# yongkyung-oh/Stable-Neural-SDEs

Measured on AMD Instinct MI355X. Metric: SDE solver steps/sec (batch x steps / s), forward solve, higher is better.
Workload: dtype f32; 1 GPU; K2: Neural LNSDE (io=4,no=17) NL=2 B=1024/GPU H=128 C=21 L=101 natural-spline coeffs 30% NaN, 100 Euler steps dt=1, ts=[0,100], in-kernel Philox dW; rows_per_gpu=1024, solver_steps=100, global_rows=1024, parallelism=row-shard x1, no collective in the solver, kernel=auto, prepare=every call (weight pack + time table launch inside the timed region, as r01-r04)

## Files before the change

stable-neural-sdes_amd/csrc/snsde_m4_kernel.h:

```cpp
#pragma once
#include <type_traits>

#include "snsde_mfma_kernels.h"

namespace snsde_mfma {

template <int H_, int NHID_, int KUXT_, int YIN_, int SAVE_, int ACT_ = 0, int ACC_ = 0>
struct CfgL {
    static constexpr bool ACC = ACC_ != 0;
    static constexpr bool SWISH = ACT_ != 0;
    static constexpr int H = H_, NHID = NHID_, KUXT = KUXT_;
    static constexpr bool YIN = YIN_ != 0;
    static constexpr bool SAVE = SAVE_ != 0;
    static constexpr int NW = H / 16;
    static constexpr int NT = NW * 64;
    static constexpr int WPS = NW >= 4 ? NW / 4 : 1;
    static constexpr int KUH = H / 16;
    static constexpr int LDY = ld_for(16 * KUH, 16);
    static constexpr int LDX = ld_for(16 * (KUXT > 0 ? KUXT : 1), 16);
    static constexpr int LDA = LDY;
    static constexpr int NLAYER = NHID + 2;
    static constexpr int NSAVE = NHID + 2 + (SWISH ? NHID + 1 : 0);
    static constexpr int ZSLOT = NHID + 1;
    static constexpr int PRE0 = NHID + 2;
    static constexpr int ZB = 4;
    static constexpr int ZSTASH = 4 * ZB * 64;
    static constexpr int ROWCH = 128;
    static constexpr int XI = KUXT > 0 ? (4 * 16 * KUXT + NT - 1) / NT : 1;
    static constexpr int RS = 8;
    static constexpr int ACCF = 64;
    static constexpr int LDS_FLOATS = 4 * (LDY + 2 * LDX + 2 * LDA) + (ROWCH + 3) * RS + NW * ZSTASH + ACCF;
};

template <bool NANZ>
__device__ __forceinline__ float lean_tanh(float x) {
    const float t = __builtin_amdgcn_exp2f(fabsf(x) * -2.8853900817779268f);
    float q = (1.0f - t) * __builtin_amdgcn_rcpf(1.0f + t);
    if constexpr (NANZ) q = __builtin_fmaxf(q, 0.0f);
    return __builtin_copysignf(q, x);
}

template <bool NANZ>
__device__ __forceinline__ float lean_tanh_rel(float x) {
    const float x2 = x * x;
    float p = fmaf(x2, -0.053968253968253971f, 0.13333333333333333f);
    p = fmaf(x2, p, -0.33333333333333333f);
    p = fmaf(x * x2, p, x);
    const float q = lean_tanh<NANZ>(x);
    return fabsf(x) < 0.125f ? p : q;
}

__device__ __forceinline__ float lean_swish(float x, float scale) {
    const float e = __builtin_amdgcn_exp2f(x * -1.4426950408889634f);
    return (x * scale) * __builtin_amdgcn_rcpf(1.0f + e);
}

template <int KU>
__device__ __forceinline__ void lean_load_w(float (&w)[KU * 4], const float* __restrict__ g, int wave, int lane) {
#pragma unroll
    for (int u = 0; u < KU; ++u) {
        const f32x4 v = *reinterpret_cast<const f32x4*>(g + (((size_t)wave * KU + u) * 64 + lane) * 4);
        w[4 * u] = v[0]; w[4 * u + 1] = v[1]; w[4 * u + 2] = v[2]; w[4 * u + 3] = v[3];
    }
}

__device__ __forceinline__ void lean_gload(float& dst, uint32_t voff, const float* sbase) {
    asm volatile("s_nop 4\n\tglobal_load_dword %0, %1, %2" : "=v"(dst) : "v"(voff), "s"(lean_uniform(sbase)) : "memory");
}
__device__ __forceinline__ void lean_gstore(float v, uint32_t voff, const float* sbase) {
    asm volatile("s_nop 4\n\tglobal_store_dword %1, %0, %2" :: "v"(v), "v"(voff), "s"(lean_uniform(sbase)));
}
__device__ __forceinline__ void lean_gload4(float& d0, float& d1, float& d2, float& d3, uint32_t v0, uint32_t v1, uint32_t v2,
                                            uint32_t v3, const float* sbase) {
    asm volatile("s_nop 4\n\tglobal_load_dword %0, %4, %8\n\tglobal_load_dword %1, %5, %8\n\tglobal_load_dword %2, %6, %8\n\t"
                 "global_load_dword %3, %7, %8"
                 : "=&v"(d0), "=&v"(d1), "=&v"(d2), "=&v"(d3) : "v"(v0), "v"(v1), "v"(v2), "v"(v3), "s"(lean_uniform(sbase)) : "memory");
}
template <int KU> struct LeanB { f32x4 v[KU]; };
__device__ __forceinline__ void lean_read_b(uint32_t a, LeanB<1>& b) {
    asm volatile("s_mov_b64 exec, 0xffff\n\tds_read_b128 %0, %[a]\n\ts_mov_b64 exec, -1" : "=&v"(b.v[0]) : [a] "v"(a));
}
__device__ __forceinline__ void lean_read_b(uint32_t a, LeanB<2>& b) {
    asm volatile("s_mov_b64 exec, 0xffff\n\tds_read_b128 %0, %[a]\n\tds_read_b128 %1, %[a] offset:64\n\ts_mov_b64 exec, -1"
                 : "=&v"(b.v[0]), "=&v"(b.v[1]) : [a] "v"(a));
}
__device__ __forceinline__ void lean_read_b(uint32_t a, LeanB<3>& b) {
    asm volatile("s_mov_b64 exec, 0xffff\n\tds_read_b128 %0, %[a]\n\tds_read_b128 %1, %[a] offset:64\n\tds_read_b128 %2, %[a] offset:128\n\t"
                 "s_mov_b64 exec, -1" : "=&v"(b.v[0]), "=&v"(b.v[1]), "=&v"(b.v[2]) : [a] "v"(a));
}
__device__ __forceinline__ void lean_read_b(uint32_t a, LeanB<4>& b) {
    asm volatile("s_mov_b64 exec, 0xffff\n\tds_read_b128 %0, %[a]\n\tds_read_b128 %1, %[a] offset:64\n\tds_read_b128 %2, %[a] offset:128\n\t"
                 "ds_read_b128 %3, %[a] offset:192\n\ts_mov_b64 exec, -1"
                 : "=&v"(b.v[0]), "=&v"(b.v[1]), "=&v"(b.v[2]), "=&v"(b.v[3]) : [a] "v"(a));
}
__device__ __forceinline__ void lean_read_b(uint32_t a, LeanB<5>& b) {
    asm volatile("s_mov_b64 exec, 0xffff\n\tds_read_b128 %0, %[a]\n\tds_read_b128 %1, %[a] offset:64\n\tds_read_b128 %2, %[a] offset:128\n\t"
                 "ds_read_b128 %3, %[a] offset:192\n\tds_read_b128 %4, %[a] offset:256\n\ts_mov_b64 exec, -1"
                 : "=&v"(b.v[0]), "=&v"(b.v[1]), "=&v"(b.v[2]), "=&v"(b.v[3]), "=&v"(b.v[4]) : [a] "v"(a));
}
__device__ __forceinline__ void lean_read_b(uint32_t a, LeanB<6>& b) {
    asm volatile("s_mov_b64 exec, 0xffff\n\tds_read_b128 %0, %[a]\n\tds_read_b128 %1, %[a] offset:64\n\tds_read_b128 %2, %[a] offset:128\n\t"
                 "ds_read_b128 %3, %[a] offset:192\n\tds_read_b128 %4, %[a] offset:256\n\tds_read_b128 %5, %[a] offset:320\n\t"
                 "s_mov_b64 exec, -1"
                 : "=&v"(b.v[0]), "=&v"(b.v[1]), "=&v"(b.v[2]), "=&v"(b.v[3]), "=&v"(b.v[4]), "=&v"(b.v[5]) : [a] "v"(a));
}
__device__ __forceinline__ void lean_read_b(uint32_t a, LeanB<8>& b) {
    asm volatile("s_mov_b64 exec, 0xffff\n\tds_read_b128 %0, %[a]\n\tds_read_b128 %1, %[a] offset:64\n\tds_read_b128 %2, %[a] offset:128\n\t"
                 "ds_read_b128 %3, %[a] offset:192\n\tds_read_b128 %4, %[a] offset:256\n\tds_read_b128 %5, %[a] offset:320\n\t"
                 "ds_read_b128 %6, %[a] offset:384\n\tds_read_b128 %7, %[a] offset:448\n\ts_mov_b64 exec, -1"
                 : "=&v"(b.v[0]), "=&v"(b.v[1]), "=&v"(b.v[2]), "=&v"(b.v[3]), "=&v"(b.v[4]), "=&v"(b.v[5]), "=&v"(b.v[6]), "=&v"(b.v[7])
                 : [a] "v"(a));
}
__device__ __forceinline__ void lean_read_b_carried(uint32_t a, LeanB<1>& b) {
    asm volatile("s_mov_b64 exec, 0xffff\n\tds_read_b128 %0, %[a]\n\ts_mov_b64 exec, -1" : "+v"(b.v[0]) : [a] "v"(a));
}
__device__ __forceinline__ void lean_read_b_carried(uint32_t a, LeanB<2>& b) {
    asm volatile("s_mov_b64 exec, 0xffff\n\tds_read_b128 %0, %[a]\n\tds_read_b128 %1, %[a] offset:64\n\ts_mov_b64 exec, -1"
                 : "+v"(b.v[0]), "+v"(b.v[1]) : [a] "v"(a));
}
__device__ __forceinline__ void lean_read_b_carried(uint32_t a, LeanB<3>& b) {
    asm volatile("s_mov_b64 exec, 0xffff\n\tds_read_b128 %0, %[a]\n\tds_read_b128 %1, %[a] offset:64\n\tds_read_b128 %2, %[a] offset:128\n\t"
                 "s_mov_b64 exec, -1" : "+v"(b.v[0]), "+v"(b.v[1]), "+v"(b.v[2]) : [a] "v"(a));
}
__device__ __forceinline__ void lean_read_b_carried(uint32_t a, LeanB<4>& b) {
    asm volatile("s_mov_b64 exec, 0xffff\n\tds_read_b128 %0, %[a]\n\tds_read_b128 %1, %[a] offset:64\n\tds_read_b128 %2, %[a] offset:128\n\t"
                 "ds_read_b128 %3, %[a] offset:192\n\ts_mov_b64 exec, -1"
                 : "+v"(b.v[0]), "+v"(b.v[1]), "+v"(b.v[2]), "+v"(b.v[3]) : [a] "v"(a));
}
__device__ __forceinline__ void lean_read_b_carried(uint32_t a, LeanB<5>& b) {
    asm volatile("s_mov_b64 exec, 0xffff\n\tds_read_b128 %0, %[a]\n\tds_read_b128 %1, %[a] offset:64\n\tds_read_b128 %2, %[a] offset:128\n\t"
                 "ds_read_b128 %3, %[a] offset:192\n\tds_read_b128 %4, %[a] offset:256\n\ts_mov_b64 exec, -1"
                 : "+v"(b.v[0]), "+v"(b.v[1]), "+v"(b.v[2]), "+v"(b.v[3]), "+v"(b.v[4]) : [a] "v"(a));
}
__device__ __forceinline__ void lean_read_b_carried(uint32_t a, LeanB<6>& b) {
    asm volatile("s_mov_b64 exec, 0xffff\n\tds_read_b128 %0, %[a]\n\tds_read_b128 %1, %[a] offset:64\n\tds_read_b128 %2, %[a] offset:128\n\t"
                 "ds_read_b128 %3, %[a] offset:192\n\tds_read_b128 %4, %[a] offset:256\n\tds_read_b128 %5, %[a] offset:320\n\t"
                 "s_mov_b64 exec, -1"
                 : "+v"(b.v[0]), "+v"(b.v[1]), "+v"(b.v[2]), "+v"(b.v[3]), "+v"(b.v[4]), "+v"(b.v[5]) : [a] "v"(a));
}
__device__ __forceinline__ void lean_read_b_carried(uint32_t a, LeanB<8>& b) {
    asm volatile("s_mov_b64 exec, 0xffff\n\tds_read_b128 %0, %[a]\n\tds_read_b128 %1, %[a] offset:64\n\tds_read_b128 %2, %[a] offset:128\n\t"
                 "ds_read_b128 %3, %[a] offset:192\n\tds_read_b128 %4, %[a] offset:256\n\tds_read_b128 %5, %[a] offset:320\n\t"
                 "ds_read_b128 %6, %[a] offset:384\n\tds_read_b128 %7, %[a] offset:448\n\ts_mov_b64 exec, -1"
                 : "+v"(b.v[0]), "+v"(b.v[1]), "+v"(b.v[2]), "+v"(b.v[3]), "+v"(b.v[4]), "+v"(b.v[5]), "+v"(b.v[6]), "+v"(b.v[7])
                 : [a] "v"(a));
}
#undef SNSDE_RD
template <int CNT> __device__ __forceinline__ void lean_wait2(f32x4& x, f32x4& y) {
    asm volatile("s_waitcnt lgkmcnt(%2)" : "+v"(x), "+v"(y) : "n"(CNT < 15 ? CNT : 15));
}
template <int CNT> __device__ __forceinline__ void lean_wait1(f32x4& x) {
    asm volatile("s_waitcnt lgkmcnt(%1)" : "+v"(x) : "n"(CNT < 15 ? CNT : 15));
}
template <int Y, int KU, int U>
__device__ __forceinline__ void lean_gemm_from(const float (&w)[KU * 4], LeanB<KU>& b, f32x4& c, f32x4& d) {
    if constexpr (U < KU) {
        if constexpr (U + 1 < KU) lean_wait2<Y + KU - 2 - U>(b.v[U], b.v[U + 1]);
        else lean_wait1<Y>(b.v[U]);
#pragma unroll
        for (int uu = U; uu < U + 2 && uu < KU; ++uu) {
            c = __builtin_amdgcn_mfma_f32_4x4x1f32(w[4 * uu], b.v[uu][0], c, 0, 0, 4);
            d = __builtin_amdgcn_mfma_f32_4x4x1f32(w[4 * uu + 1], b.v[uu][1], d, 0, 0, 4);
            c = __builtin_amdgcn_mfma_f32_4x4x1f32(w[4 * uu + 2], b.v[uu][2], c, 0, 0, 4);
            d = __builtin_amdgcn_mfma_f32_4x4x1f32(w[4 * uu + 3], b.v[uu][3], d, 0, 0, 4);
        }
        __builtin_amdgcn_sched_barrier(0);
        lean_gemm_from<Y, KU, U + 2>(w, b, c, d);
    }
}
template <int Y, int KU>
__device__ __forceinline__ void lean_gemm(const float (&w)[KU * 4], LeanB<KU>& b, f32x4& c, f32x4& d) {
    lean_gemm_from<Y, KU, 0>(w, b, c, d);
}

typedef short s16x4 __attribute__((ext_vector_type(4)));
typedef __bf16 bf16x4 __attribute__((ext_vector_type(4)));
template <class CF> struct CfgBf16 : CF { static constexpr bool BF = true; };
template <class CF, class = void> struct lean_bf : std::false_type {};
template <class CF> struct lean_bf<CF, std::void_t<decltype(CF::BF)>> : std::bool_constant<CF::BF> {};
template <int KU> struct LeanBh { s16x4 v[KU]; };
template <bool BF, int KU> using LeanWt = std::conditional_t<BF, s16x4[KU], float[KU * 4]>;
template <bool BF, int KU> using LeanBt = std::conditional_t<BF, LeanBh<KU>, LeanB<KU>>;
template <bool BF> using LeanOp = std::conditional_t<BF, __bf16, float>;

__device__ __forceinline__ s16x4 lean_bf16x4(f32x4 v) {
    const bf16x4 b = {(__bf16)v[0], (__bf16)v[1], (__bf16)v[2], (__bf16)v[3]};
    return __builtin_bit_cast(s16x4, b);
}
template <int KU>
__device__ __forceinline__ void lean_load_w(s16x4 (&w)[KU], const float* __restrict__ g, int wave, int lane) {
#pragma unroll
    for (int u = 0; u < KU; ++u) w[u] = lean_bf16x4(*reinterpret_cast<const f32x4*>(g + (((size_t)wave * KU + u) * 64 + lane) * 4));
}
template <bool BF>
__device__ __forceinline__ uint32_t lean_op_addr(const float* buf, int roff, int col) {
    if constexpr (BF) return lean_lds_addr(buf) + (uint32_t)((roff + col) * 2);
    else return lean_lds_addr(buf + roff + col);
}
#define LEAN_RB(i, o) "\n\tds_read_b64 %" #i ", %[a] offset:" #o
#define LEAN_RB_PRE "s_mov_b64 exec, 0xffff"
#define LEAN_RB_POST "\n\ts_mov_b64 exec, -1"
__device__ __forceinline__ void lean_read_b(uint32_t a, LeanBh<1>& b) {
    asm volatile(LEAN_RB_PRE LEAN_RB(0, 0) LEAN_RB_POST : "=&v"(b.v[0]) : [a] "v"(a));
}
__device__ __forceinline__ void lean_read_b(uint32_t a, LeanBh<2>& b) {
    asm volatile(LEAN_RB_PRE LEAN_RB(0, 0) LEAN_RB(1, 32) LEAN_RB_POST : "=&v"(b.v[0]), "=&v"(b.v[1]) : [a] "v"(a));
}
__device__ __forceinline__ void lean_read_b(uint32_t a, LeanBh<3>& b) {
    asm volatile(LEAN_RB_PRE LEAN_RB(0, 0) LEAN_RB(1, 32) LEAN_RB(2, 64) LEAN_RB_POST
                 : "=&v"(b.v[0]), "=&v"(b.v[1]), "=&v"(b.v[2]) : [a] "v"(a));
}
__device__ __forceinline__ void lean_read_b(uint32_t a, LeanBh<4>& b) {
    asm volatile(LEAN_RB_PRE LEAN_RB(0, 0) LEAN_RB(1, 32) LEAN_RB(2, 64) LEAN_RB(3, 96) LEAN_RB_POST
                 : "=&v"(b.v[0]), "=&v"(b.v[1]), "=&v"(b.v[2]), "=&v"(b.v[3]) : [a] "v"(a));
}
__device__ __forceinline__ void lean_read_b(uint32_t a, LeanBh<6>& b) {
    asm volatile(LEAN_RB_PRE LEAN_RB(0, 0) LEAN_RB(1, 32) LEAN_RB(2, 64) LEAN_RB(3, 96) LEAN_RB(4, 128) LEAN_RB(5, 160) LEAN_RB_POST
                 : "=&v"(b.v[0]), "=&v"(b.v[1]), "=&v"(b.v[2]), "=&v"(b.v[3]), "=&v"(b.v[4]), "=&v"(b.v[5]) : [a] "v"(a));
}
__device__ __forceinline__ void lean_read_b(uint32_t a, LeanBh<8>& b) {
    asm volatile(LEAN_RB_PRE LEAN_RB(0, 0) LEAN_RB(1, 32) LEAN_RB(2, 64) LEAN_RB(3, 96) LEAN_RB(4, 128) LEAN_RB(5, 160)
                 LEAN_RB(6, 192) LEAN_RB(7, 224) LEAN_RB_POST
                 : "=&v"(b.v[0]), "=&v"(b.v[1]), "=&v"(b.v[2]), "=&v"(b.v[3]), "=&v"(b.v[4]), "=&v"(b.v[5]), "=&v"(b.v[6]),
                   "=&v"(b.v[7]) : [a] "v"(a));
}
__device__ __forceinline__ void lean_read_b_carried(uint32_t a, LeanBh<1>& b) {
    asm volatile(LEAN_RB_PRE LEAN_RB(0, 0) LEAN_RB_POST : "+v"(b.v[0]) : [a] "v"(a));
}
__device__ __forceinline__ void lean_read_b_carried(uint32_t a, LeanBh<2>& b) {
    asm volatile(LEAN_RB_PRE LEAN_RB(0, 0) LEAN_RB(1, 32) LEAN_RB_POST : "+v"(b.v[0]), "+v"(b.v[1]) : [a] "v"(a));
}
__device__ __forceinline__ void lean_read_b_carried(uint32_t a, LeanBh<3>& b) {
    asm volatile(LEAN_RB_PRE LEAN_RB(0, 0) LEAN_RB(1, 32) LEAN_RB(2, 64) LEAN_RB_POST
                 : "+v"(b.v[0]), "+v"(b.v[1]), "+v"(b.v[2]) : [a] "v"(a));
}
__device__ __forceinline__ void lean_read_b_carried(uint32_t a, LeanBh<6>& b) {
    asm volatile(LEAN_RB_PRE LEAN_RB(0, 0) LEAN_RB(1, 32) LEAN_RB(2, 64) LEAN_RB(3, 96) LEAN_RB(4, 128) LEAN_RB(5, 160) LEAN_RB_POST
                 : "+v"(b.v[0]), "+v"(b.v[1]), "+v"(b.v[2]), "+v"(b.v[3]), "+v"(b.v[4]), "+v"(b.v[5]) : [a] "v"(a));
}
#undef LEAN_RB
#undef LEAN_RB_PRE
#undef LEAN_RB_POST
template <int CNT> __device__ __forceinline__ void lean_wait2(s16x4& x, s16x4& y) {
    asm volatile("s_waitcnt lgkmcnt(%2)" : "+v"(x), "+v"(y) : "n"(CNT < 15 ? CNT : 15));
}
template <int CNT> __device__ __forceinline__ void lean_wait1(s16x4& x) {
    asm volatile("s_waitcnt lgkmcnt(%1)" : "+v"(x) : "n"(CNT < 15 ? CNT : 15));
}
template <int Y, int KU, int U>
__device__ __forceinline__ void lean_gemm_from(const s16x4 (&w)[KU], LeanBh<KU>& b, f32x4& c, f32x4& d) {
    if constexpr (U < KU) {
        if constexpr (U + 1 < KU) lean_wait2<Y + KU - 2 - U>(b.v[U], b.v[U + 1]);
        else lean_wait1<Y>(b.v[U]);
        c = __builtin_amdgcn_mfma_f32_4x4x4bf16_1k(w[U], b.v[U], c, 0, 0, 4);
        if constexpr (U + 1 < KU) d = __builtin_amdgcn_mfma_f32_4x4x4bf16_1k(w[U + 1], b.v[U + 1], d, 0, 0, 4);
        __builtin_amdgcn_sched_barrier(0);
        lean_gemm_from<Y, KU, U + 2>(w, b, c, d);
    }
}
template <int Y, int KU>
__device__ __forceinline__ void lean_gemm(const s16x4 (&w)[KU], LeanBh<KU>& b, f32x4& c, f32x4& d) {
    lean_gemm_from<Y, KU, 0>(w, b, c, d);
}

template <class CF, int GEO_> struct CfgSpec : CF {
    static constexpr bool SPEC = true, SPEC_GEO = GEO_ != 0;
    static constexpr int XB = 4;
    static constexpr int LDS_FLOATS = CF::LDS_FLOATS + 4 * (XB - 2) * CF::LDX;
    static_assert(CF::XI == 1 && 4 * 16 * CF::KUXT <= 16 * CF::NW && CF::ROWCH % XB == 0, "CfgSpec: one spline entry per lane, 16 lanes per step of a batch");
};
template <class CF, class = void> struct lean_spec : std::false_type {};
template <class CF> struct lean_spec<CF, std::void_t<decltype(CF::SPEC)>> : std::bool_constant<CF::SPEC> {};
template <class CF> constexpr int lean_xslots() {
    if constexpr (lean_spec<CF>::value) return CF::XB;
    else return 2;
}
template <class CF> constexpr bool lean_spec_geo() {
    if constexpr (lean_spec<CF>::value) return CF::SPEC_GEO;
    else return false;
}

#ifdef LEAN_TRACE
#define LT_DECL unsigned long long lt[10]; uint32_t* const ltl = reinterpret_cast<uint32_t*>(lds + CF::LDS_FLOATS) + tid; \
    if constexpr (!BF) { for (int i_ = 0; i_ < 12; ++i_) ltl[i_ * NT] = 0u; }
#define LT(i) if constexpr (!BF) { asm volatile("s_memtime %0" : "=s"(lt[i])); }
#define LT_ADD(slot, i) __hip_atomic_fetch_add(ltl + (slot) * NT, (uint32_t)lt[i], __ATOMIC_RELAXED, __HIP_MEMORY_SCOPE_WORKGROUP);
#define LT_COLLECT_A if constexpr (!BF) { asm volatile("s_waitcnt lgkmcnt(0)" : "+s"(lt[0]), "+s"(lt[1]), "+s"(lt[2]), "+s"(lt[3])); \
    LT_ADD(0, 0) LT_ADD(1, 1) LT_ADD(2, 2) LT_ADD(3, 3) if (n > 0) LT_ADD(10, 0) }
#define LT_COLLECT_B if constexpr (!BF) { asm volatile("s_waitcnt lgkmcnt(0)" : "+s"(lt[4]), "+s"(lt[5]), "+s"(lt[6])); LT_ADD(4, 4) LT_ADD(5, 5) LT_ADD(6, 6) }
#define LT_COLLECT if constexpr (!BF) { asm volatile("s_waitcnt lgkmcnt(0)" : "+s"(lt[7]), "+s"(lt[8]), "+s"(lt[9])); LT_ADD(7, 7) LT_ADD(8, 8) LT_ADD(9, 9) \
    if (n + 1 < N) LT_ADD(11, 9) }
#define LT_LDS_EXTRA (12 * CF::NT * sizeof(uint32_t))
#else
#define LT_DECL
#define LT(i)
#define LT_COLLECT_A
#define LT_COLLECT_B
#define LT_COLLECT
#define LT_LDS_EXTRA 0
#endif

#ifdef LEAN_KNOCKOUT
#define LEAN_KO(SP) (SP)
#else
#define LEAN_KO(SP) false
#endif
#if (defined(LEAN_KNOCKOUT) || defined(LEAN_SPEC_WPS)) && !defined(SNSDE_DEV_SUBSET)
#error "LEAN_KNOCKOUT / LEAN_SPEC_WPS are development switches (build.py variant): never part of a product build"
#endif
#ifndef LEAN_SPEC_WPS
#define LEAN_SPEC_WPS CF::WPS
#endif

#ifndef LEAN_TANH_F
#define LEAN_TANH_F lean_tanh_rel<false>
#endif
#ifndef LEAN_TANH_G
#define LEAN_TANH_G lean_tanh_rel<true>
#endif

template <class CF>
__global__ void __launch_bounds__(CF::NT, lean_spec<CF>::value ? LEAN_SPEC_WPS : CF::WPS) snsde_m4_kernel(MfmaArgs a) {
    constexpr int H = CF::H, NT = CF::NT, NHID = CF::NHID, KUH = CF::KUH, KUXT = CF::KUXT;
    constexpr int LDY = CF::LDY, LDX = CF::LDX, LDA = CF::LDA, RS = CF::RS;
    constexpr bool YIN = CF::YIN, SAVE = CF::SAVE;
    constexpr bool BF = lean_bf<CF>::value;
    constexpr bool SP = lean_spec<CF>::value;
    static_assert(!SP || (!BF && !CF::ACC && !CF::SWISH && KUXT > 0 && 16 * KUXT + 16 <= LDX), "CfgSpec: f32 relu fields with a control path");
    using OpT = LeanOp<BF>;
    extern __shared__ __attribute__((aligned(16))) float lds[];
    float* ybuf = lds;
    constexpr int XS = lean_xslots<CF>();
    float* xbuf = ybuf + 4 * LDY;
    float* bufA = xbuf + 4 * XS * LDX;
    float* bufB = bufA + 4 * LDA;
    float* rowtab = bufB + 4 * LDA;
    float* zstash_all = rowtab + (CF::ROWCH + 3) * RS;
    float* accbuf = zstash_all + CF::NW * CF::ZSTASH;

    const int tid = threadIdx.x;
    const int lane = tid & 63;
    const int wave = __builtin_amdgcn_readfirstlane(tid >> 6);
    const int r = lane & 3, s = (lane >> 2) & 3, q = lane >> 4;
    const int fo = wave * 16 + 4 * q + s;
    const int row0 = blockIdx.x * 4;
    const int B = a.B, C = a.C, N = a.N;
    const int row = row0 + r;
    const bool row_ok = row < B;
    const int rowc = row_ok ? row : B - 1;
    const size_t BH = (size_t)B * H;
    const size_t goff = (size_t)rowc * H + fo;
    float* zstash = zstash_all + wave * CF::ZSTASH;
    const uint32_t fo4 = (uint32_t)(fo * sizeof(float)), goff4 = (uint32_t)(goff * sizeof(float));
    const int xc = a.lean_xc;
    const bool time_on = a.lean_time != 0, geo = SP ? lean_spec_geo<CF>() : a.lean_geo != 0;
    const float act_scale = a.act == SNSDE_ACT_LIPSWISH ? 0.909f : 1.0f;
    const int f_out = SP ? (int)SNSDE_DRIFT_TANH : a.f_out;
    const bool g_raw = !SP && a.g_out == SNSDE_DIFFUSION_RAW;

    int li = 0;
    LeanWt<BF, (KUXT > 0 ? KUXT : 1)> wxt;
    LeanWt<BF, KUH> wy, wh[NHID > 0 ? NHID : 1], wo;
    if constexpr (KUXT > 0) lean_load_w<KUXT>(wxt, a.ws + a.w_off[li++], wave, lane);
    if constexpr (YIN) lean_load_w<KUH>(wy, a.ws + a.w_off[li++], wave, lane);
#pragma unroll
    for (int l = 0; l < NHID; ++l) lean_load_w<KUH>(wh[l], a.ws + a.w_off[li++], wave, lane);
    lean_load_w<KUH>(wo, a.ws + a.w_off[li++], wave, lane);
    f32x4 bfr[CF::NLAYER];
#pragma unroll
    for (int l = 0; l < CF::NLAYER; ++l)
#pragma unroll
        for (int i = 0; i < 4; ++i) bfr[l][i] = (s == 0) ? a.ws[a.bias_off + l * H + wave * 16 + 4 * q + i] : 0.0f;

    for (int i = tid; i < 4 * (LDY + XS * LDX + 2 * LDA); i += NT) lds[i] = 0.0f;
    auto fill_rows = [&](int base) {
        for (int i = tid; i < (CF::ROWCH + 3) * RS; i += NT) {
            const int j = i % RS;
            int rr = base + i / RS + (j == 0 ? 0 : (j == 7 ? 2 : 1));
            rr = rr < N - 1 ? rr : N - 1;
            const int src = j == 0 ? 1 : j == 1 ? 6 : j == 4 ? (a.raw_time ? 0 : 2) : j == 5 ? (a.raw_time ? 10 : 3) : j == 6 ? 4 : j == 7 ? 5 : 10;
            rowtab[i] = a.step_tab[(size_t)rr * SNSDE_STEP_STRIDE + src];
        }
    };
    fill_rows(0);
    __syncthreads();

    const float sig_theta = snsde_sigmoid(a.params[a.off_theta]);
    const int no = a.no;
    const bool tab = SP || a.gt_off >= 0;
    const float* gt = a.gt_ext ? a.gt_ext : a.ws + (tab ? a.gt_off : 0);
    const bool mul_y = SP || (no == 13 || no == 17 || no == 3 || no == 6 || no == 11);
    const bool yfun = !SP && (no >= 7 && no <= 10);
    const bool mil = !SP && a.method == SNSDE_MILSTEIN;
    const bool phx = SP || a.dW == nullptr;
    const uint32_t grow = (uint32_t)(a.row_offset + row);
    const uint64_t seed = a.seed_dev ? *a.seed_dev : a.seed;
    const int rslot = a.row_out ? a.row_out[rowc] : -1;

    float yv = a.y0[goff];
    reinterpret_cast<OpT*>(ybuf)[r * LDY + fo] = (OpT)yv;
    if (row_ok) {
        a.ys[(size_t)row * H + fo] = yv;
        if constexpr (SAVE) { if (a.traj) a.traj[(size_t)row * H + fo] = yv; }
    }

    const int xw = xc + (time_on ? 2 : 0);
    const int xquota = (4 * xw + CF::NW - 1) / CF::NW;
    float ca[CF::XI], cb[CF::XI], cc[CF::XI], cd[CF::XI];
    uint32_t cvo[CF::XI];
    int xdst[CF::XI], xkind[CF::XI];
    const size_t cstride = (size_t)(a.L - 1) * 4 * C;
    [[maybe_unused]] const int xslot = SP ? ((1 + q) & 3) * (4 * LDX) : 0;
#pragma unroll
    for (int i = 0; i < CF::XI; ++i) {
        const int li_ = SP ? (lane & 15) : lane + 64 * i, it = wave * xquota + li_;
        const bool ok = KUXT > 0 && li_ < xquota && it < 4 * xw;
        const int rr = ok ? it / xw : 0, col = ok ? it - rr * xw : 0;
        xdst[i] = ok ? rr * LDX + col : (SP ? (lane & 3) * LDX + 16 * KUXT + (lane >> 2) : -1);
        xkind[i] = col < xc ? 0 : (col == xc ? 1 : 2);
        const int gr = row0 + rr < B ? rr : B - 1 - row0, ch = col < xc ? col : 0;
        cvo[i] = (uint32_t)((gr * cstride + ch) * sizeof(float));
    }
    const bool has_x = SP || (KUXT > 0 && xc > 0);
    const float* ctile = a.coeffs + (size_t)row0 * cstride;
    const uint32_t cstep = (uint32_t)(C * sizeof(float));
    const uint32_t cidx = (uint32_t)(4 * C * sizeof(float));
    auto load_coeffs = [&](int idx) {
        if (__builtin_expect(has_x, 1)) {
            const uint32_t io = (uint32_t)idx * cidx;
#pragma unroll
            for (int i = 0; i < CF::XI; ++i)
                lean_gload4(ca[i], cb[i], cc[i], cd[i], cvo[i] + io, cvo[i] + io + cstep, cvo[i] + io + 2 * cstep,
                            cvo[i] + io + 3 * cstep, ctile);
        }
    };
    auto vm_wait = [&](float& dwn, float& gtn) {
        asm volatile("s_waitcnt vmcnt(0)" : "+v"(dwn), "+v"(gtn));
#pragma unroll
        for (int i = 0; i < CF::XI; ++i) asm volatile("" : "+v"(ca[i]), "+v"(cb[i]), "+v"(cc[i]), "+v"(cd[i]));
    };
    auto store_xt = [&](float* xb, float frac, float sn, float cs) {
        if constexpr (KUXT > 0) {
#pragma unroll
            for (int i = 0; i < CF::XI; ++i) {
                float v = 0.0f;
                if (__builtin_expect(has_x, 1)) {
                    const float x3 = cd[i] * frac;
                    float q3 = x3 * 0.333333343f;
                    q3 = fmaf(fmaf(-3.0f, q3, x3), 0.333333343f, q3);
                    v = ca[i] + (cb[i] + (0.5f * cc[i] + q3) * frac) * frac;
                }
                v = xkind[i] == 0 ? v : (xkind[i] == 1 ? sn : cs);
                if (SP || xdst[i] >= 0) reinterpret_cast<OpT*>(xb)[xdst[i]] = (OpT)v;
            }
        }
    };

    auto next_dw = [&](int i, float sqh) -> float {
        if (__builtin_expect(phx, 1)) {
            const int k = (int)((uint32_t)i % (uint32_t)(4 * CF::ZB));
            if (__builtin_expect(k == 0 && !(LEAN_KO(SP) && i > 0), 0)) {
                float zq[4 * CF::ZB];
#pragma unroll
                for (int bb = 0; bb < CF::ZB; ++bb)
                    snsde_philox_normal4(seed, grow, (uint32_t)((i >> 2) + bb), (uint32_t)fo, &zq[4 * bb]);
#pragma unroll
                for (int j = 0; j < 4 * CF::ZB; ++j) zstash[j * 64 + lane] = zq[j];
            }
            return zstash[k * 64 + lane] * sqh;
        }
        float v;
        lean_gload(v, goff4, a.dW + (size_t)i * BH);
        return v;
    };

    auto gpart = [&](float y, float gtv, float dwv, float hh) -> float {
        float g = 0.0f, draw = 0.0f;
        if (__builtin_expect(yfun, 0)) {
            float p1, p2;
            const float raw = snsde_phi(no, y, p1, p2);
            g = fast_tanh(sig_theta * snsde_nan_to_num(raw));
            draw = snsde_finite(raw) ? p1 : 0.0f;
        } else
        {
            const float raw = mul_y ? gtv * y : gtv;
            if (__builtin_expect(g_raw, 0)) {
                float yp = fmaf(raw, dwv, y);
                if (mil && mul_y) yp = fmaf(0.5f * raw * gtv, fmaf(dwv, dwv, -hh), yp);
                return yp;
            }
            g = LEAN_TANH_G(sig_theta * raw);
            draw = (mul_y && snsde_finite(raw)) ? gtv : 0.0f;
        }
        float yp = fmaf(g, dwv, y);
        if (__builtin_expect(mil, 0)) yp = fmaf(0.5f * (g * ((1.0f - g * g) * sig_theta * draw)), fmaf(dwv, dwv, -hh), yp);
        return yp;
    };

    float dw_cur, gt_cur = 0.0f;
    f32x4 qa, qb;
    {
        const float* g0 = a.step_tab;
        load_coeffs(__float_as_int(g0[5]));
        float dummy = 0.0f;
        vm_wait(dummy, gt_cur);
        store_xt(xbuf, g0[4], a.raw_time ? g0[0] : g0[2], a.raw_time ? 0.0f : g0[3]);
        dw_cur = next_dw(0, g0[6]);
        if (tab) lean_gload(gt_cur, fo4, gt);
        if constexpr (SP) {
            const int m = 1 + q < N - 1 ? 1 + q : N - 1;
            load_coeffs(__float_as_int(a.step_tab[(size_t)m * SNSDE_STEP_STRIDE + 5]));
        } else
        load_coeffs(__float_as_int(a.step_tab[(size_t)(N > 1 ? 1 : 0) * SNSDE_STEP_STRIDE + 5]));
        vm_wait(dw_cur, gt_cur);
        qa = *reinterpret_cast<const f32x4*>(rowtab);
        qb = *reinterpret_cast<const f32x4*>(rowtab + 4);
    }
    __syncthreads();
#ifndef LEAN_PRIO_MODE
#define LEAN_PRIO_MODE 1
#endif
    if constexpr (LEAN_PRIO_MODE == 1) { if (__builtin_amdgcn_readfirstlane(tid) >= NT / 2 && CF::NW >= 8) __builtin_amdgcn_s_setprio(1); }
    if constexpr (LEAN_PRIO_MODE == 2) { if (__builtin_amdgcn_readfirstlane(tid) < NT / 2 && CF::NW >= 8) __builtin_amdgcn_s_setprio(1); }

    const uint32_t yrow = lean_op_addr<BF>(ybuf, r * LDY, 4 * s);
    const uint32_t xrow = lean_op_addr<BF>(xbuf, r * LDX, 4 * s);
    const uint32_t arow = lean_op_addr<BF>(bufA, r * LDA, 4 * s);
    const uint32_t brow = lean_op_addr<BF>(bufB, r * LDA, 4 * s);
    OpT* const aown = reinterpret_cast<OpT*>(bufA) + r * LDA + fo;
    OpT* const bown = reinterpret_cast<OpT*>(bufB) + r * LDA + fo;
    const f32x4 zero4 = {0.f, 0.f, 0.f, 0.f};

    LeanBt<BF, (KUXT > 0 ? KUXT : 1)> bx{};
    if constexpr (KUXT > 0) lean_read_b_carried(xrow, bx);
    if constexpr (SP) {
        if constexpr (KUXT == 1) asm volatile("s_waitcnt lgkmcnt(0)" : "+v"(bx.v[0]));
        else asm volatile("s_waitcnt lgkmcnt(0)" : "+v"(bx.v[0]), "+v"(bx.v[1]));
        static_assert(KUXT <= 2, "tie every fragment of bx to the wait");
        __syncthreads();
    }
    LT_DECL
    int n = 0;
    float yold = yv;
    for (int ko = 0; ko < a.T - 1; ++ko) {
    const int n_end = a.out_step[ko];
    for (; n <= n_end; ++n) {
        const int rbase = (n / CF::ROWCH) * CF::ROWCH;
        if (n > 0 && n == rbase) {
            fill_rows(rbase);
            __syncthreads();
        }
        const bool more = n + 1 < N;
        [[maybe_unused]] float* act_n = nullptr;
        [[maybe_unused]] uint32_t nu = 0;
        [[maybe_unused]] uint32_t sgn = 0;
        if constexpr (SAVE) {
            nu = (uint32_t)__builtin_amdgcn_readfirstlane(n);
            act_n = a.act_save + uoff((int)nu, (uint32_t)CF::NSAVE * (uint32_t)BH);
        }
        LT(0)
        LeanBt<BF, KUH> by;
        if constexpr (YIN) lean_read_b(yrow, by);
        asm volatile("" : "+v"(qa), "+v"(qb));
        const float h = qa[0];
        __builtin_amdgcn_sched_barrier(0);
        f32x4 c = bfr[0], d = zero4;
        if constexpr (KUXT > 0) lean_gemm<15, KUXT>(wxt, bx, c, d);
        const float ypart = gpart(yv, gt_cur, dw_cur, h);
        if constexpr (SP) {
            if constexpr (!LEAN_KO(SP)) {
                if ((n & (CF::XB - 1)) == 0) {
                    const float* rp = rowtab + (n - rbase + q) * RS;
                    const f32x4 qk = *reinterpret_cast<const f32x4*>(rp + 4);
                    const float ik = rp[3 * RS + 7];
                    store_xt(xbuf + xslot, qk[2], qk[0], qk[1]);
                    load_coeffs(__float_as_int(ik));
                }
            }
        } else {
            store_xt(xbuf + ((n + 1) & 1) * (4 * LDX), qb[2], qb[0], qb[1]);
            load_coeffs(__float_as_int(qb[3]));
        }
        __builtin_amdgcn_sched_barrier(0);
        LT(1)
        if constexpr (YIN) lean_gemm<0, KUH>(wy, by, c, d);
        LT(2)
        {
            const float pre = m4_reduce_scatter(c + d);
            const float o = CF::SWISH ? lean_swish(pre, act_scale) : fmaxf(pre, 0.0f);
            *aown = (OpT)o;
            if constexpr (SAVE) {
                if (a.act_save && row_ok) {
                    lean_gstore(o, goff4, act_n);
                    if constexpr (CF::SWISH) lean_gstore(pre, goff4, act_n + uoff(0, 0, CF::PRE0, (uint32_t)BH));
                }
                if constexpr (!CF::SWISH) sgn = o > 0.0f ? 1u : 0u;
            }
        }
        LT(3)
        __syncthreads();
        LT_COLLECT_A
        LT(4)
        float dw_nxt = 0.0f, gt_nxt = 0.0f;
        auto prep = [&]() {
            {
                const int n1 = more ? n + 1 : n;
                dw_nxt = next_dw(n1, qa[1]);
                if (__builtin_expect(tab, 1)) lean_gload(gt_nxt, fo4, gt + (size_t)(uint32_t)__builtin_amdgcn_readfirstlane(n1) * H);
            }
        };
        uint32_t cur = arow;
#pragma unroll
        for (int l = 0; l < NHID; ++l) {
            const bool toB = (l % 2 == 0);
            LeanBt<BF, KUH> bh;
            lean_read_b(cur, bh);
            __builtin_amdgcn_sched_barrier(0);
            if (l == 0) prep();
            __builtin_amdgcn_sched_barrier(0);
            if (l == 0) { LT(5) }
            c = bfr[1 + l]; d = zero4;
            lean_gemm<0, KUH>(wh[l], bh, c, d);
            const float pre = m4_reduce_scatter(c + d);
            const float o = CF::SWISH ? lean_swish(pre, act_scale) : fmaxf(pre, 0.0f);
            *(toB ? bown : aown) = (OpT)o;
            if constexpr (SAVE) {
                if (a.act_save && row_ok) {
                    lean_gstore(o, goff4, act_n + uoff(0, 0, 1 + l, (uint32_t)BH));
                    if constexpr (CF::SWISH) lean_gstore(pre, goff4, act_n + uoff(0, 0, CF::PRE0 + 1 + l, (uint32_t)BH));
                }
                if constexpr (!CF::SWISH) sgn |= (o > 0.0f ? 1u : 0u) << (1 + l);
            }
            if (l == NHID - 1) { LT(6) }
            __syncthreads();
            if (l == NHID - 1) { LT_COLLECT_B LT(7) }
            cur = toB ? brow : arow;
        }
        {
            LeanBt<BF, KUH> bo;
            lean_read_b(cur, bo);
            __builtin_amdgcn_sched_barrier(0);
            if (NHID == 0) prep();
            __builtin_amdgcn_sched_barrier(0);
            c = bfr[NHID + 1]; d = zero4;
            lean_gemm<0, KUH>(wo, bo, c, d);
        }
        LT(8)
        vm_wait(dw_nxt, gt_nxt);
        float z = m4_reduce_scatter(c + d);
        if constexpr (SAVE) {
            if (a.act_save && row_ok) lean_gstore(CF::SWISH ? z : snsde_pack_signs(z, sgn, NHID + 1), goff4, act_n + uoff(0, 0, CF::ZSLOT, (uint32_t)BH));
        }
        if (__builtin_expect(geo, 0)) z *= fast_tanh(yv);
        float f;
        if (__builtin_expect(f_out != SNSDE_DRIFT_TANH, 0)) f = f_out == SNSDE_DRIFT_TIMES_Y ? z * yv : z;
        else f = LEAN_TANH_F(z);
        if constexpr (CF::ACC) {
            if (__builtin_expect(a.acc_col >= 0, 0)) {
                float ev = 0.0f;
                if (fo < a.acc_col) {
                    const float qv = (f - fmaf(a.acc_a, yv, a.acc_b)) * snsde_stable_inv(gt_cur);
                    ev = 0.5f * qv * qv;
                }
                ev = m4_row_sum(ev);
                if (lane < 4) accbuf[wave * 4 + lane] = ev;
                __syncthreads();
                if (fo == a.acc_col) {
                    float u = 0.0f;
                    for (int w = 0; w < CF::NW; ++w) u += accbuf[w * 4 + r];
                    f = u;
                }
            }
        }
        const float ynew = fmaf(f, h, ypart);
        yold = yv;
        yv = ynew;
        reinterpret_cast<OpT*>(ybuf)[r * LDY + fo] = (OpT)ynew;
        if constexpr (SAVE) {
            if (row_ok) {
                if (a.traj) lean_gstore(ynew, goff4, a.traj + uoff((int)nu + 1, (uint32_t)BH));
                if (a.dW_out) lean_gstore(dw_cur, goff4, a.dW_out + uoff((int)nu, (uint32_t)BH));
            }
        }
        dw_cur = dw_nxt; gt_cur = gt_nxt;
        asm volatile("ds_read_b128 %0, %2\n\tds_read_b128 %1, %2 offset:16"
                     : "+v"(qa), "+v"(qb) : "v"(lean_lds_addr(rowtab + (n + 1 - rbase) * RS)));
        if constexpr (KUXT > 0) lean_read_b_carried(xrow + ((n + 1) & (XS - 1)) * (4 * LDX * 4), bx);
        LT(9)
        __syncthreads();
        LT_COLLECT
    }
    if (row_ok) {
        const float w0 = a.out_w[2 * ko], w1 = a.out_w[2 * ko + 1];
        const float o = (w0 == 0.0f) ? yv : snsde_interp_out(w0, w1, yold, yv);
        if (!a.row_out) a.ys[(size_t)(ko + 1) * BH + goff] = o;
        else if (rslot == ko + 1) a.ys[goff] = o;
    }
    }
#ifdef LEAN_TRACE
    __syncthreads();
    if (blockIdx.x == 0 && lane == 0) {
        float* o = a.ys + (a.row_out ? 0 : (size_t)(a.T - 1) * BH);
        o[wave * 16] = (float)(uint32_t)(ltl[10 * NT] - ltl[11 * NT]);
        for (int i = 1; i < 10; ++i) o[wave * 16 + i] = (float)(uint32_t)(ltl[i * NT] - ltl[(i - 1) * NT]);
    }
#endif
}

template <class CF>
int launch_lean(const MfmaArgs& a, hipStream_t stream) {
    const size_t lds_bytes = (size_t)CF::LDS_FLOATS * sizeof(float) + LT_LDS_EXTRA;
    static SnsdeLdsAttr lds_attr;
    if (const int rc = snsde_lds_attr(reinterpret_cast<const void*>(snsde_m4_kernel<CF>), lds_bytes, lds_attr)) return rc;
    const int grid = (a.B + 3) / 4;
    hipLaunchKernelGGL(snsde_m4_kernel<CF>, dim3(grid), dim3(CF::NT), lds_bytes, stream, a);
    return hipGetLastError() == hipSuccess ? SNSDE_OK : SNSDE_ERR_LAUNCH;
}

#define SNSDE_LEAN_SPEC_LIST(X) X(128, 1, 2)
__host__ __device__ constexpr bool lean_spec_instantiated(int h, int nhid, int kuxt) {
#define SNSDE_LEAN_SPEC_HAS(H_, NH_, KX_) if (h == H_ && nhid == NH_ && kuxt == KX_) return true;
    SNSDE_LEAN_SPEC_LIST(SNSDE_LEAN_SPEC_HAS)
#undef SNSDE_LEAN_SPEC_HAS
    return false;
}

template <int H>
int dispatch_lean(const MfmaPlan& p, const MfmaArgs& a, hipStream_t st) {
    const bool save = a.act_save || a.traj || a.dW_out;
    if (p.LEAN_SPEC) {
#define SNSDE_LEAN_SPEC_CASE(H_, NH_, KX_) \
        if constexpr (H == H_) { if (p.NHID == NH_ && p.KUXT == KX_) { \
            if (p.LEAN_SPEC == 2) return save ? launch_lean<CfgSpec<CfgL<H_, NH_, KX_, 1, 1>, 1>>(a, st) \
                                              : launch_lean<CfgSpec<CfgL<H_, NH_, KX_, 1, 0>, 1>>(a, st); \
            return save ? launch_lean<CfgSpec<CfgL<H_, NH_, KX_, 1, 1>, 0>>(a, st) : launch_lean<CfgSpec<CfgL<H_, NH_, KX_, 1, 0>, 0>>(a, st); } }
        SNSDE_LEAN_SPEC_LIST(SNSDE_LEAN_SPEC_CASE)
#undef SNSDE_LEAN_SPEC_CASE
        return SNSDE_ERR_UNSUPPORTED;
    }
    if (a.acc_col >= 0) {
#ifndef SNSDE_DEV_SUBSET
#define SNSDE_LEAN_ACC(NH_) \
    if constexpr (lean_fits(H, NH_, 1, true) && lean_act_save_fits(H, NH_, 1)) { \
        if (p.NHID == NH_ && p.KUXT == 1 && p.IO != 0 && a.act == SNSDE_ACT_RELU) \
            return save ? launch_lean<CfgL<H, NH_, 1, 1, 1, 0, 1>>(a, st) : launch_lean<CfgL<H, NH_, 1, 1, 0, 0, 1>>(a, st); }
        SNSDE_LEAN_ACC(0) SNSDE_LEAN_ACC(1) SNSDE_LEAN_ACC(2) SNSDE_LEAN_ACC(3)
#undef SNSDE_LEAN_ACC
#endif
        return SNSDE_ERR_UNSUPPORTED;
    }
    if (a.act != SNSDE_ACT_RELU) {
#define SNSDE_LEAN_ACT(NH_, KX_) \
    if constexpr (lean_fits(H, NH_, KX_, true)) { \
        if (p.NHID == NH_ && p.KUXT == KX_ && p.IO != 0) { \
            if (!save) return launch_lean<CfgL<H, NH_, KX_, 1, 0, 1>>(a, st); \
            if constexpr (lean_act_save_fits(H, NH_, KX_)) return launch_lean<CfgL<H, NH_, KX_, 1, 1, 1>>(a, st); \
            else return SNSDE_ERR_UNSUPPORTED; } }
#ifndef SNSDE_DEV_SUBSET
        SNSDE_LEAN_ACT(0, 1) SNSDE_LEAN_ACT(1, 1) SNSDE_LEAN_ACT(2, 1) SNSDE_LEAN_ACT(3, 1)
        SNSDE_LEAN_ACT(0, 2) SNSDE_LEAN_ACT(1, 2) SNSDE_LEAN_ACT(2, 2) SNSDE_LEAN_ACT(3, 2)
        SNSDE_LEAN_ACT(0, 3) SNSDE_LEAN_ACT(1, 3) SNSDE_LEAN_ACT(2, 3) SNSDE_LEAN_ACT(3, 3)
#endif
#undef SNSDE_LEAN_ACT
        return SNSDE_ERR_UNSUPPORTED;
    }
#ifdef SNSDE_DEV_SUBSET
    if (p.NHID == 1 && p.KUXT == 2 && p.IO != 0)
        return save ? launch_lean<CfgL<H, 1, 2, 1, 1>>(a, st) : launch_lean<CfgL<H, 1, 2, 1, 0>>(a, st);
    if (p.NHID == 1 && p.KUXT == 1 && p.IO != 0)
        return save ? launch_lean<CfgL<H, 1, 1, 1, 1>>(a, st) : launch_lean<CfgL<H, 1, 1, 1, 0>>(a, st);
    return SNSDE_ERR_UNSUPPORTED;
#else
#define SNSDE_LEAN(NH_, KX_, Y_) \
    if constexpr (lean_fits(H, NH_, KX_, Y_ != 0)) { \
        if (p.NHID == NH_ && p.KUXT == KX_ && (p.IO != 0) == (Y_ != 0)) \
            return save ? launch_lean<CfgL<H, NH_, KX_, Y_, 1>>(a, st) : launch_lean<CfgL<H, NH_, KX_, Y_, 0>>(a, st); }
#define SNSDE_LEANS(KX_, Y_) SNSDE_LEAN(0, KX_, Y_) SNSDE_LEAN(1, KX_, Y_) SNSDE_LEAN(2, KX_, Y_) SNSDE_LEAN(3, KX_, Y_)
    SNSDE_LEANS(0, 1) SNSDE_LEANS(1, 1) SNSDE_LEANS(2, 1) SNSDE_LEANS(3, 1) SNSDE_LEANS(6, 1)
    SNSDE_LEANS(1, 0) SNSDE_LEANS(2, 0) SNSDE_LEANS(3, 0) SNSDE_LEANS(6, 0)
#undef SNSDE_LEANS
#undef SNSDE_LEAN
    return SNSDE_ERR_UNSUPPORTED;
#endif
}

int dispatch_lean_h32(const MfmaPlan& p, const MfmaArgs& a, hipStream_t st);
int dispatch_lean_h64(const MfmaPlan& p, const MfmaArgs& a, hipStream_t st);
int dispatch_lean_h128(const MfmaPlan& p, const MfmaArgs& a, hipStream_t st);
int dispatch_lean_h128_two_tile(const MfmaPlan& p, const MfmaArgs& a, hipStream_t st);
int dispatch_lean_h256(const MfmaPlan& p, const MfmaArgs& a, hipStream_t st);
int dispatch_lean_h256_two_tile(const MfmaPlan& p, const MfmaArgs& a, hipStream_t st);
int dispatch_lean_bf16_h64(const MfmaPlan& p, const MfmaArgs& a, hipStream_t st);
int dispatch_lean_bf16_h128(const MfmaPlan& p, const MfmaArgs& a, hipStream_t st);
bool m4t_instantiated(int nhid, int kuxt, bool save);
bool m4s2_instantiated(int nhid, int kuxt, bool save);

}
```

Before: 594.5 million row-steps/s.

## Shadow next step's control GEMM and diffusion term into the previous step

Adds a LEAN_SHADOW_MODE switch, defaulting to 2, for the speculative lean kernel. In this mode the next step's control-path GEMM (wxt·x) is computed during the current step's output-layer block. The diffusion part `gpart` is computed just before the end-of-step barrier, so neither sits at the head of the next step's critical path. This trades extra live accumulator registers, and a reordered LDS read of the next x slot, for shorter dependent latency per step. The loop-body `gpart` call passes h=0 where the original passed the step size, which is a correctness risk if gpart depends on h. The trace instrumentation also gains one more timestamp slot.

```diff
diff --git a/stable-neural-sdes_amd/csrc/snsde_m4_kernel.h b/stable-neural-sdes_amd/csrc/snsde_m4_kernel.h
--- a/stable-neural-sdes_amd/csrc/snsde_m4_kernel.h
+++ b/stable-neural-sdes_amd/csrc/snsde_m4_kernel.h
@@ -281,16 +281,16 @@
 }
 
 #ifdef LEAN_TRACE
-#define LT_DECL unsigned long long lt[10]; uint32_t* const ltl = reinterpret_cast<uint32_t*>(lds + CF::LDS_FLOATS) + tid; \
-    if constexpr (!BF) { for (int i_ = 0; i_ < 12; ++i_) ltl[i_ * NT] = 0u; }
+#define LT_DECL unsigned long long lt[11]; uint32_t* const ltl = reinterpret_cast<uint32_t*>(lds + CF::LDS_FLOATS) + tid; \
+    if constexpr (!BF) { for (int i_ = 0; i_ < 13; ++i_) ltl[i_ * NT] = 0u; }
 #define LT(i) if constexpr (!BF) { asm volatile("s_memtime %0" : "=s"(lt[i])); }
 #define LT_ADD(slot, i) __hip_atomic_fetch_add(ltl + (slot) * NT, (uint32_t)lt[i], __ATOMIC_RELAXED, __HIP_MEMORY_SCOPE_WORKGROUP);
 #define LT_COLLECT_A if constexpr (!BF) { asm volatile("s_waitcnt lgkmcnt(0)" : "+s"(lt[0]), "+s"(lt[1]), "+s"(lt[2]), "+s"(lt[3])); \
-    LT_ADD(0, 0) LT_ADD(1, 1) LT_ADD(2, 2) LT_ADD(3, 3) if (n > 0) LT_ADD(10, 0) }
+    LT_ADD(0, 0) LT_ADD(1, 1) LT_ADD(2, 2) LT_ADD(3, 3) if (n > 0) LT_ADD(11, 0) }
 #define LT_COLLECT_B if constexpr (!BF) { asm volatile("s_waitcnt lgkmcnt(0)" : "+s"(lt[4]), "+s"(lt[5]), "+s"(lt[6])); LT_ADD(4, 4) LT_ADD(5, 5) LT_ADD(6, 6) }
-#define LT_COLLECT if constexpr (!BF) { asm volatile("s_waitcnt lgkmcnt(0)" : "+s"(lt[7]), "+s"(lt[8]), "+s"(lt[9])); LT_ADD(7, 7) LT_ADD(8, 8) LT_ADD(9, 9) \
-    if (n + 1 < N) LT_ADD(11, 9) }
-#define LT_LDS_EXTRA (12 * CF::NT * sizeof(uint32_t))
+#define LT_COLLECT if constexpr (!BF) { asm volatile("s_waitcnt lgkmcnt(0)" : "+s"(lt[7]), "+s"(lt[8]), "+s"(lt[9]), "+s"(lt[10])); \
+    LT_ADD(7, 7) LT_ADD(8, 8) LT_ADD(9, 9) LT_ADD(10, 10) if (n + 1 < N) LT_ADD(12, 10) }
+#define LT_LDS_EXTRA (13 * CF::NT * sizeof(uint32_t))
 #else
 #define LT_DECL
 #define LT(i)
@@ -312,6 +312,9 @@
 #define LEAN_SPEC_WPS CF::WPS
 #endif
 
+#ifndef LEAN_SHADOW_MODE
+#define LEAN_SHADOW_MODE 2
+#endif
 #ifndef LEAN_TANH_F
 #define LEAN_TANH_F lean_tanh_rel<false>
 #endif
@@ -326,6 +329,8 @@
     constexpr bool YIN = CF::YIN, SAVE = CF::SAVE;
     constexpr bool BF = lean_bf<CF>::value;
     constexpr bool SP = lean_spec<CF>::value;
+    constexpr bool SH1 = SP && LEAN_SHADOW_MODE >= 1;
+    constexpr bool SH2 = SP && LEAN_SHADOW_MODE >= 2;
     static_assert(!SP || (!BF && !CF::ACC && !CF::SWISH && KUXT > 0 && 16 * KUXT + 16 <= LDX), "CfgSpec: f32 relu fields with a control path");
     using OpT = LeanOp<BF>;
     extern __shared__ __attribute__((aligned(16))) float lds[];
@@ -533,10 +538,14 @@
 
     LeanBt<BF, (KUXT > 0 ? KUXT : 1)> bx{};
     if constexpr (KUXT > 0) lean_read_b_carried(xrow, bx);
+    [[maybe_unused]] f32x4 cx = zero4, dx = zero4;
+    [[maybe_unused]] float ypart_c = 0.0f;
     if constexpr (SP) {
         if constexpr (KUXT == 1) asm volatile("s_waitcnt lgkmcnt(0)" : "+v"(bx.v[0]));
         else asm volatile("s_waitcnt lgkmcnt(0)" : "+v"(bx.v[0]), "+v"(bx.v[1]));
         static_assert(KUXT <= 2, "tie every fragment of bx to the wait");
+        if constexpr (SH2) { cx = bfr[0]; lean_gemm<0, KUXT>(wxt, bx, cx, dx); }
+        if constexpr (SH1) ypart_c = gpart(yv, gt_cur, dw_cur, qa[0]);
         __syncthreads();
     }
     LT_DECL
@@ -565,8 +574,11 @@
         const float h = qa[0];
         __builtin_amdgcn_sched_barrier(0);
         f32x4 c = bfr[0], d = zero4;
-        if constexpr (KUXT > 0) lean_gemm<15, KUXT>(wxt, bx, c, d);
-        const float ypart = gpart(yv, gt_cur, dw_cur, h);
+        if constexpr (SH2) { c = cx; d = dx; }
+        else if constexpr (KUXT > 0) lean_gemm<15, KUXT>(wxt, bx, c, d);
+        float ypart;
+        if constexpr (SH1) ypart = ypart_c;
+        else ypart = gpart(yv, gt_cur, dw_cur, h);
         if constexpr (SP) {
             if constexpr (!LEAN_KO(SP)) {
                 if ((n & (CF::XB - 1)) == 0) {
@@ -638,10 +650,13 @@
         }
         {
             LeanBt<BF, KUH> bo;
+            [[maybe_unused]] LeanBt<BF, (KUXT > 0 ? KUXT : 1)> bxn;
+            if constexpr (SH2) lean_read_b(xrow + ((n + 1) & (XS - 1)) * (4 * LDX * 4), bxn);
             lean_read_b(cur, bo);
             __builtin_amdgcn_sched_barrier(0);
             if (NHID == 0) prep();
             __builtin_amdgcn_sched_barrier(0);
+            if constexpr (SH2) { cx = bfr[0]; dx = zero4; lean_gemm<KUH, KUXT>(wxt, bxn, cx, dx); }
             c = bfr[NHID + 1]; d = zero4;
             lean_gemm<0, KUH>(wo, bo, c, d);
         }
@@ -685,8 +700,14 @@
         dw_cur = dw_nxt; gt_cur = gt_nxt;
         asm volatile("ds_read_b128 %0, %2\n\tds_read_b128 %1, %2 offset:16"
                      : "+v"(qa), "+v"(qb) : "v"(lean_lds_addr(rowtab + (n + 1 - rbase) * RS)));
-        if constexpr (KUXT > 0) lean_read_b_carried(xrow + ((n + 1) & (XS - 1)) * (4 * LDX * 4), bx);
+        if constexpr (KUXT > 0 && !SH2) lean_read_b_carried(xrow + ((n + 1) & (XS - 1)) * (4 * LDX * 4), bx);
         LT(9)
+        if constexpr (SH1) {
+            __builtin_amdgcn_sched_barrier(0);
+            ypart_c = gpart(yv, gt_cur, dw_cur, 0.0f);
+            __builtin_amdgcn_sched_barrier(0);
+        }
+        LT(10)
         __syncthreads();
         LT_COLLECT
     }
@@ -701,8 +722,8 @@
     __syncthreads();
     if (blockIdx.x == 0 && lane == 0) {
         float* o = a.ys + (a.row_out ? 0 : (size_t)(a.T - 1) * BH);
-        o[wave * 16] = (float)(uint32_t)(ltl[10 * NT] - ltl[11 * NT]);
-        for (int i = 1; i < 10; ++i) o[wave * 16 + i] = (float)(uint32_t)(ltl[i * NT] - ltl[(i - 1) * NT]);
+        o[wave * 16] = (float)(uint32_t)(ltl[11 * NT] - ltl[12 * NT]);
+        for (int i = 1; i < 11; ++i) o[wave * 16 + i] = (float)(uint32_t)(ltl[i * NT] - ltl[(i - 1) * NT]);
     }
 #endif
 }
```

Result: slower. 583.5 million row-steps/s (-1.8%).
